# wreuven/h264-scroll-encoder

Hardware: AMD Instinct MI355X
Metric: composed frames/sec (1280x720, 360x360 dyn) at 1/2/4/8 GPU; bit-exact vs CPU (higher is better)
Workload: dtype u8; 1 GPU; BASELINE config 3: 256 concurrent 1280x720 streams + 360x360 synthetic dynamic rect (4x4 int transform + quant + CAVLC), composer_write_scroll_frame semantics; resolution=1280x720, streams_per_gpu=256, parallelism=static stream shard x1, no RCCL

## Files before the change

h264-scroll-encoder_amd/csrc/dyn_device.h:

```cpp
#ifndef SCROLL_DYN_DEVICE_H
#define SCROLL_DYN_DEVICE_H

#include "qparams.h"
#include "scroll_device.h"

namespace scroll {
namespace dyn {

constexpr int QP_DEFAULT = 26, QP_MIN = 22, QP_MAX = 51, LEVEL_MAX = 2063;
__host__ __device__ constexpr int mf_of(int r, int cls)
{
    constexpr int T[6][3] = {{13107, 5243, 8066}, {11916, 4660, 7490}, {10082, 4194, 6554},
                             {9362, 3647, 5825},  {8192, 3355, 5243},  {7282, 2893, 4559}};
    return T[r][cls];
}
__host__ __device__ constexpr QParams qparams(int qp)
{
    return QParams{mf_of(qp % 6, 0), mf_of(qp % 6, 1), mf_of(qp % 6, 2), 15 + qp / 6, (1 << (15 + qp / 6)) / 6};
}
__device__ __host__ inline QParams qparams_rt(int qp)
{
    const int r = qp % 6, b = 15 + qp / 6;
    const int m0 = r == 0 ? 13107 : r == 1 ? 11916 : r == 2 ? 10082 : r == 3 ? 9362 : r == 4 ? 8192 : 7282;
    const int m1 = r == 0 ? 5243 : r == 1 ? 4660 : r == 2 ? 4194 : r == 3 ? 3647 : r == 4 ? 3355 : 2893;
// ... 984 lines not shown
    uint32_t m = (t1 == 0 ? g0 : (t1 == 1 ? g1 : (t1 == 2 ? g2 : g3))) >> 1;
    auto push = [](uint64_t &ac, uint32_t &n, uint32_t v, uint32_t len, CAP &c) {
        if (n + len > 64u) {
            if (n > 32u) c.put((uint32_t)(ac >> 32), (int)(n - 32u));
            c.put((uint32_t)ac, n > 32u ? 32 : (int)n);
            ac = 0;
            n = 0;
        }
        ac = (ac << len) | v;
        n += len;
    };
    int cls = ((tc > 10 && t1 < 3) ? 1 : 0) + (t1 < 3 ? 7 : 0);
    auto level_code = [&](int v, int cl) -> uint32_t {
        if (v >= -LVT_V && v <= LVT_V) return lvt[cl * LVT_W + v + LVT_V + 1];
        const int sl = cl >= 7 ? cl - 7 : cl, adj = cl >= 7 ? 2 : 0;
        const int a = v < 0 ? -v : v;
        const int code = 2 * a - 2 + (v < 0 ? 1 : 0) - adj;
        const int lim = sl ? (15 << sl) : 30;
        const uint32_t mk = (1u << sl) - 1u;
        uint32_t fv = ((uint32_t)code & mk) | (mk + 1u);
        uint32_t fl = (uint32_t)((code >> sl) + 1 + sl);
        const bool e15 = code >= lim, e14 = sl == 0 && code >= 14;
        fv = e15 ? (uint32_t)(4096 + code - lim) : (e14 ? (uint32_t)(code + 2) : fv);
        fl = e15 ? 28u : (e14 ? 19u : fl);
        const int s1 = sl == 0 ? 1 : sl;
        return fv | fl << 13 | (uint32_t)(s1 + ((a > (3 << (s1 - 1)) && s1 < 6) ? 1 : 0)) << 18;
    };
#ifndef SCROLL_CAVLC_NOPF
    const uint32_t m0 = m, an0 = an;
    const uint64_t acc0 = acc;
    const int cls0 = cls;
    const CAP cap0 = cap;
    bool big = false;
    int pn = top_bit(m);
    int vn = (int)lb[pn ^ (int)bx];
    for (int k = t1; k < tc; ++k) {
        const int v = vn;
        m &= ~(1u << pn);
        pn = top_bit(m);
        vn = (int)lb[pn ^ (int)bx];
        const int vc = v < -LVT_V ? -LVT_V : (v > LVT_V ? LVT_V : v);
        big |= vc != v;
        const uint32_t e = lvt[cls * LVT_W + vc + LVT_V + 1];
        push(acc, an, e & 0x1fffu, (e >> 13) & 31u, cap);
        cls = (int)(e >> 18);
    }
    if (big) {
        m = m0;
        an = an0;
        acc = acc0;
        cls = cls0;
        cap = cap0;
        for (int k = t1; k < tc; ++k) {
            const int p = top_bit(m);
            m &= ~(1u << p);
            const uint32_t e = level_code((int)lb[p ^ (int)bx], cls);
            push(acc, an, e & 0x1fffu, (e >> 13) & 31u, cap);
            cls = (int)(e >> 18);
        }
    }
#else
    for (int k = t1; k < tc; ++k) {
        const int p = top_bit(m);
        m &= ~(1u << p);
        const uint32_t e = level_code((int)lb[p ^ (int)bx], cls);
        push(acc, an, e & 0x1fffu, (e >> 13) & 31u, cap);
        cls = (int)(e >> 18);
    }
#endif
    const uint32_t tzl = 31u - (uint32_t)__builtin_ctz(tzrb);
    push(acc, an, (tzrb >> 1) >> (31u - tzl), tzl, cap);
    if (cap.n == 0) {
        cap.lo = acc;
        cap.n = an;
        return tc;
    }
    if (an > 32u) cap.put((uint32_t)(acc >> 32), (int)(an - 32u));
    cap.put((uint32_t)acc, an > 32u ? 32 : (int)an);
    ok = cap.n <= 128;
    return tc;
}

template <class CAP, class PT>
__device__ __host__ inline int cavlc_dc4(CAP &cap, const PT &P, const int c[4])
{
    const uint32_t nz = (c[0] != 0 ? 1u : 0u) | (c[1] != 0 ? 2u : 0u) | (c[2] != 0 ? 4u : 0u) |
                        (c[3] != 0 ? 8u : 0u);
    const int tc = __builtin_popcount(nz);
    int t1 = 0;
    bool trail = true;
#pragma unroll
    for (int i = 3; i >= 0; --i) {
        const bool one = c[i] == 1 || c[i] == -1;
        if (c[i] != 0) {
            trail = trail && one && t1 < 3;
            t1 += trail ? 1 : 0;
        }
    }
    {
        const uint32_t e = P.ct[3][4 * tc + t1];
        cap.put(e & 255u, (int)(e >> 8));
    }
    if (tc == 0) return 0;
    int k = 0, sl = 0, zl = 0, pprev = -1;
    uint64_t runs = 0;
    int rn = 0;
    const int hi = top_bit(nz);
    const int tz = hi + 1 - tc;
    zl = tz;
#pragma unroll
    for (int i = 3; i >= 0; --i) {
        const int v = c[i];
        if (v != 0) {
            const int a = v < 0 ? -v : v;
            if (k < t1) {
                cap.put(v < 0 ? 1u : 0u, 1);
            } else {
                int code = 2 * a - 2 + (v < 0 ? 1 : 0);
                if (k == t1 && t1 < 3) code -= 2;
                uint32_t fv;
                int fl;
                level_field_bf(code, sl, fv, fl);
                cap.put(fv, fl);
                if (sl == 0) sl = 1;
                if (a > (3 << (sl - 1)) && sl < 6) sl++;
            }
            if (k > 0 && zl > 0) {
                const int run = pprev - i - 1;
                const uint32_t e = P.rb[(zl < 7 ? zl : 7) - 1][run];
                runs = (runs << (e >> 8)) | (e & 255u);
                rn += (int)(e >> 8);
                zl -= run;
            }
            pprev = i;
            k++;
        }
    }
    if (tc < 4) {
        const uint32_t e = P.tzdc[tc - 1][tz];
        cap.put(e & 255u, (int)(e >> 8));
    }
    cap.put((uint32_t)runs, rn);
    return tc;
}

__device__ __host__ inline bool ep_insert(uint32_t b, int k) { return b <= 3 && k >= 2 && !(k & 1); }

__device__ __host__ inline int blk_raster(int blk)
{
    const int q8 = blk >> 2, q4 = blk & 3;
    return 4 * ((q8 >> 1) * 2 + (q4 >> 1)) + (q8 & 1) * 2 + (q4 & 1);
}

struct Rect {
    int x0, y0, w, h;
};

__device__ __host__ inline uint32_t magic32(uint32_t d) { return d <= 1 ? 0u : 0xffffffffu / d + 1u; }
__device__ __host__ inline uint32_t div_m(uint32_t x, uint32_t m) { return m ? __umulhi(x, m) : x; }
__device__ __host__ inline uint32_t magic16(uint32_t d) { return (65536u + d - 1u) / d; }
__device__ __host__ inline uint32_t div16(uint32_t x, uint32_t m16) { return __umul24(x, m16) >> 16; }

__device__ __host__ inline int dyn_rank(const Rect &r, int mbw, int m)
{
    const int y = m / mbw, x = m - y * mbw;
    if (y < r.y0) return 0;
    if (y >= r.y0 + r.h) return r.w * r.h;
    return (y - r.y0) * r.w + clampi(x - r.x0, 0, r.w);
}

__device__ __host__ inline int dyn_rank_m(const Rect &r, int mbw, uint32_t m_mbw, int m)
{
    const int y = (int)div_m((uint32_t)m, m_mbw), x = m - y * mbw;
    if (y < r.y0) return 0;
    if (y >= r.y0 + r.h) return r.w * r.h;
    return (y - r.y0) * r.w + clampi(x - r.x0, 0, r.w);
}

__device__ __host__ inline int dyn_mb_m(const Rect &r, int mbw, uint32_t m_rw, int q)
{
    const int ry = (int)div_m((uint32_t)q, m_rw);
    return (r.y0 + ry) * mbw + r.x0 + (q - ry * r.w);
}

__device__ __host__ inline int dyn_mb(const Rect &r, int mbw, int q)
{
    const int ry = q / r.w;
    return (r.y0 + ry) * mbw + r.x0 + (q - ry * r.w);
}

}
}
#endif
```

h264-scroll-encoder_amd/csrc/dyn_kernels.hip:

```cpp
#include <hip/hip_runtime.h>

#include <stdint.h>
#include <mutex>

#include "dyn_device.h"
#include "dyn_engine.h"
#include "nal_ctx.h"
#include "row_mfma.h"
#include "stage_util.h"

using namespace scroll;
using namespace scroll::dyn;
using namespace scroll::stage;

namespace {

__constant__ Tabs g_tabs = SCROLL_DYN_TABS;
constexpr Tabs k_tabs = SCROLL_DYN_TABS;
__constant__ PTabs g_ptabs = make_ptabs(k_tabs);
__device__ uint32_t g_tzrb[TZRB_N];
__constant__ LvTab g_lvt = make_lvt();

struct QpPair {
    QParams l, c;
// ... 376 lines not shown
        const uint16_t mm = ok ? (uint16_t)(cap.n | (uint32_t)tc << 8 | (uint32_t)t1 << 13)
                               : (uint16_t)((uint32_t)tc << 8 | (uint32_t)t1 << 13 | M_OVF);
        M[tk] = mm;
        uint4 ov = v4;
        if (wide && !ok) {
            const uint4 *l2 = reinterpret_cast<const uint4 *>(lw[u]);
            ov = l2[0];
            BW[tk] = l2[1];
        }
        if ((mm & 255u) || (mm & M_OVF))
            put_body(BL, BH, tk,
                     ok ? make_uint4((uint32_t)cap.lo, (uint32_t)(cap.lo >> 32), (uint32_t)cap.hi,
                                     (uint32_t)(cap.hi >> 32))
                        : ov,
                     (mm & 255u) > 64u || (mm & M_OVF));
    }
}

#ifndef SCROLL_CODE_GEN_Y
#define SCROLL_CODE_GEN_Y 64
#endif
constexpr int CODE_GEN_Y = SCROLL_CODE_GEN_Y;
__global__ __launch_bounds__(CODE_T) void k_dyn_code_general(const DevStream *__restrict__ st,
                                                             const DynFrame *__restrict__ dfr, int ld_fr,
                                                             const PlanPending *__restrict__ pend,
                                                             const NalDesc *__restrict__ nal, int ld_nal,
                                                             DynGeom g, const uint32_t *__restrict__ rows,
                                                             const uint8_t *__restrict__ src,
                                                             const uint8_t *__restrict__ refs,
                                                             uint16_t *__restrict__ meta,
                                                             uint2 *__restrict__ blo, uint2 *__restrict__ bhi,
                                                             uint4 *__restrict__ bwd, const uint32_t *__restrict__ ctr)
{
    const uint32_t n = min(__builtin_amdgcn_readfirstlane(ctr[1]), g.gen_cap);
    for (uint32_t j = blockIdx.y; j < n; j += gridDim.y) {
        const uint32_t q = __builtin_amdgcn_readfirstlane(ctr[DYN_CTR_LIST + j]);
        const int s = (int)(q / (uint32_t)ld_fr), f = (int)(q - (uint32_t)s * (uint32_t)ld_fr);
        code_frame(st, dfr, ld_fr, pend, nal, ld_nal, g, rows, src, refs, meta, blo, bhi, bwd, s, f, blockIdx.x);
        __syncthreads();
    }
}

struct LdsOrWin {
    uint32_t *b;
    uint32_t lo, n;
    __device__ inline void operator()(uint32_t i, uint32_t v) const
    {
        const uint32_t k = i - lo;
        if (k < n) atomicOr(&b[k], v);
    }
};
typedef OrSink<LdsOrWin> WSink;


__device__ inline int tc_of(uint32_t m) { return (int)((m >> 8) & 31u); }

struct HeadCtx {
    Regions rg;
    int a_end, mbw, nrefs;
    __device__ inline int sel(int row, int col) const
    {
        const bool curA = row < a_end, abvA = (row - 1) < a_end;
        return 3 * (row == 0 ? 0 : (curA ? 1 : (abvA ? 2 : 3))) + (col == 0 ? 0 : (col == mbw - 1 ? 2 : 1));
    }
    template <class S>
    __device__ inline void put_class(S &sk, int cls) const
    {
        const int ty = cls / 3, pos = cls - 3 * ty;
        const int x = pos == 0 ? 0 : (pos == 1 ? min(1, mbw - 1) : mbw - 1);
        const bool cur = ty == 0 ? 0 < a_end : ty == 1;
        const bool abv = ty == 1 || ty == 2;
        const int ref = cur ? rg.ra : rg.rb, mv4 = 4 * (cur ? rg.mva : rg.mvb);
        const int aref = abv ? rg.ra : rg.rb, amv4 = 4 * (abv ? rg.mva : rg.mvb);
        int px, py;
        predict(x, ty == 0 ? 0 : 1, mbw, ref, mv4, aref, amv4, px, py);
        put_mb_head(sk, ref, 0 - px, mv4 - py, nrefs);
    }
    template <class S>
    __device__ inline void put_slow(S &sk, int row, int col) const
    {
        const bool curA = row < a_end, abvA = (row - 1) < a_end;
        const int ref = curA ? rg.ra : rg.rb, mv4 = 4 * (curA ? rg.mva : rg.mvb);
        const int aref = abvA ? rg.ra : rg.rb, amv4 = 4 * (abvA ? rg.mva : rg.mvb);
        int px, py;
        predict(col, row, mbw, ref, mv4, aref, amv4, px, py);
        put_mb_head(sk, ref, 0 - px, mv4 - py, nrefs);
    }
};

__device__ inline HeadCtx head_ctx(const NalCtx &c)
{
    HeadCtx H;
    H.rg = regions(c);
    H.a_end = (c.h - c.off) / 16;
    H.mbw = c.w / 16;
    H.nrefs = 2 + c.nwp;
    return H;
}

__device__ inline uint32_t row_static_bits(const HeadCtx &H, const uint32_t *hlen, int row, const Rect &R)
{
    const int mbw = H.mbw;
    const bool in = row >= R.y0 && row < R.y0 + R.h;
    auto isdyn = [&](int col) { return in && col >= R.x0 && col < R.x0 + R.w; };
    const int base = H.sel(row, 0) - 0;
    uint32_t bits = isdyn(0) ? 0u : hlen[base] + 1u;
    if (mbw >= 2) {
        if (!isdyn(mbw - 1)) bits += hlen[base + 2] + 1u;
        int nmid = mbw - 2;
        if (in) nmid -= max(0, min(R.x0 + R.w, mbw - 1) - max(R.x0, 1));
        bits += (uint32_t)nmid * (hlen[base + 1] + 1u);
    }
    return bits;
}

__device__ inline void lb_store(unsigned long long *p, uint64_t v)
{
    __hip_atomic_store(p, v, __ATOMIC_RELAXED, __HIP_MEMORY_SCOPE_AGENT);
}

__host__ __device__ inline uint64_t rs_group_words(const DynGeom &g, int nA, int gi)
{
    if (gi < nA) return (uint64_t)gi * g.rs_static_words;
    if (gi < nA + g.h) return (uint64_t)nA * g.rs_static_words + (uint64_t)(gi - nA) * g.rs_row_words;
    return (uint64_t)(gi - g.h) * g.rs_static_words + (uint64_t)g.h * g.rs_row_words;
}

__host__ __device__ inline uint64_t rs_runs_words(const DynGeom &g, int nA, int gi)
{
    const bool row = gi >= nA && gi < nA + g.h;
    return rs_group_words(g, nA, gi) + (row ? g.rs_row_words - EPC_ROW : g.rs_static_words - EPC_STATIC);
}

constexpr uint32_t LO_LEN = 0x7ffu;

__device__ inline void piece_token(const uint16_t (*ct)[68], uint32_t mv, int nC, uint32_t &tv, uint32_t &tl)
{
    const int tc = tc_of(mv), t1 = (int)((mv >> 13) & 3u);
    if (nC >= 8) {
        tv = tc ? (uint32_t)(((tc - 1) << 2) | t1) : 3u;
        tl = 6;
    } else {
        const uint32_t e = ct[nC < 2 ? 0 : (nC < 4 ? 1 : 2)][4 * tc + t1];
        tv = e & 255u;
        tl = e >> 8;
    }
}

__device__ inline void wave_sync()
{
    __builtin_amdgcn_fence(__ATOMIC_RELEASE, "wavefront");
    __builtin_amdgcn_wave_barrier();
    __builtin_amdgcn_fence(__ATOMIC_ACQUIRE, "wavefront");
}

template <class S>
__device__ inline void ovf_code(S &sk, const PTabs &PT, const Tabs &TB, uint4 bd, const uint4 *bw, int pc, int nC)
{
    if (nC == -1) {
        const int dq[4] = {(int)(int16_t)(bd.x & 0xffffu), (int)(int16_t)(bd.x >> 16),
                           (int)(int16_t)(bd.y & 0xffffu), (int)(int16_t)(bd.y >> 16)};
        cavlc_dc4(sk, PT, dq);
    } else if (bw) {
        const uint4 hi = *bw;
        const uint32_t w8[8] = {bd.x, bd.y, bd.z, bd.w, hi.x, hi.y, hi.z, hi.w};
        int16_t l16[16];
#pragma unroll
        for (int i = 0; i < 8; ++i) {
            l16[2 * i] = (int16_t)(w8[i] & 0xffffu);
            l16[2 * i + 1] = (int16_t)(w8[i] >> 16);
        }
        cavlc_block(sk, TB, l16, pc < 16 ? 16 : 15, nC);
    } else {
        const int8_t *lvp = reinterpret_cast<const int8_t *>(&bd);
        cavlc_block(sk, TB, lvp, pc < 16 ? 16 : 15, nC);
    }
}

__device__ __attribute__((noinline)) uint32_t ovf_bits(const PTabs &PT, const Tabs &TB, uint4 bd, const uint4 *bw,
                                                       int pc, int nC)
{
    CountSink cn{0};
    ovf_code(cn, PT, TB, bd, bw, pc, nC);
    return cn.n;
}

__device__ __attribute__((noinline)) void ovf_put(uint32_t *buf, uint32_t lo, uint32_t n, uint32_t pos,
                                                  const PTabs &PT, const Tabs &TB, uint4 bd, const uint4 *bw, int pc,
                                                  int nC)
{
    WSink sk{LdsOrWin{buf, lo, n}, 0, 0, 0};
    sk.start(pos);
    ovf_code(sk, PT, TB, bd, bw, pc, nC);
    sk.finish();
}

__device__ inline uint4 body_msb(uint64_t hi, uint64_t lo, uint32_t n)
{
    const uint32_t k = 128u - n;
    uint64_t H, Lw;
    if (k >= 64u) {
        H = k >= 128u ? 0ull : lo << (k - 64u);
        Lw = 0ull;
    } else {
        H = k ? (hi << k) | (lo >> (64u - k)) : hi;
        Lw = lo << k;
    }
    return make_uint4((uint32_t)(H >> 32), (uint32_t)H, (uint32_t)(Lw >> 32), (uint32_t)Lw);
}

__global__ __launch_bounds__(256) void k_dyn_rows(const DevStream *__restrict__ st,
                                                  const NalDesc *__restrict__ nal, int ld_nal,
                                                  const PlanPending *__restrict__ pend,
                                                  DynFrame *__restrict__ dfr, int ld_fr, DynGeom g,
                                                  uint32_t *__restrict__ rows, uint32_t *__restrict__ ctr,
                                                  uint4 *__restrict__ heads)
{
    __shared__ int32_t wo[8], wl[8], wv[8];
    __shared__ int32_t gen;
    const int s = blockIdx.y, f = blockIdx.x, t = threadIdx.x;
    DynFrame *DF = dfr + (size_t)s * ld_fr + f;
    const int j = DF->nal;
    if (j < 0) return;
    if (t < 8) {
        wo[t] = pend[s].wo[t];
        wl[t] = pend[s].wl[t];
        wv[t] = pend[s].wv[t];
    }
    if (t == 0) gen = 0;
    __syncthreads();
    const DevStream *S = st + s;
    const NalDesc d = nal[(size_t)s * ld_nal + j];
    const NalCtx c = nal_ctx(S, d, wo, wl, wv);
    if (t < 12) {
        const HeadCtx H = head_ctx(c);
        CapSink hc{0, 0, 0};
        H.put_class(hc, t);
        uint4 *hv = heads + ((size_t)s * ld_fr + f) * DYN_HEAD_VECS;
        hv[t] = body_msb(hc.hi, hc.lo, min(hc.n, 128u));
        reinterpret_cast<uint32_t *>(hv + 12)[t] = hc.n | (hc.over() ? 0x80000000u : 0u);
    }
    const Regions rg = regions(c);
    const int w = c.w, h = c.h, a_end = (h - c.off) / 16;
    const uint32_t ysz = (uint32_t)w * (uint32_t)h, pic = ysz + ysz / 2;
    const WpTab T{wo, wv, h};
    uint32_t *rw = rows + ((size_t)s * ld_fr + f) * (size_t)(32 * g.h);
    bool my_gen = false;
    for (int i = t; i < 32 * g.h; i += 256) {
        uint32_t e;
        if (i < 16 * g.h) {
            const int Y = 16 * g.y0 + i, row = Y >> 4;
            const bool cA = row < a_end;
            int yo;
            const int b = luma_row(T, cA ? rg.ra : rg.rb, Y + (cA ? rg.mva : rg.mvb), yo);
            e = (uint32_t)b * pic + (uint32_t)yo * (uint32_t)w;
        } else {
            const int i2 = i - 16 * g.h, bot = i2 >= 8 * g.h;
            const int Y = 8 * g.y0 + (bot ? i2 - 8 * g.h : i2), row = Y >> 3;
            const bool cA = row < a_end;
            const int q = 4 * (cA ? rg.mva : rg.mvb), o = q >> 3, fr = q & 7;
            int yo;
            const int b = chroma_row(T, cA ? rg.ra : rg.rb, Y + o + bot, yo);
            if (b < 0) {
                e = ROW_GEN;
                if (!bot || fr) my_gen = true;
            } else {
                e = ((uint32_t)b * pic + ysz + (uint32_t)yo * (uint32_t)(w / 2)) | (uint32_t)fr << 28;
            }
        }
        rw[i] = e;
    }
    if (my_gen || S->dyn_qp < QP_MIN) gen = 1;
    __syncthreads();
    if (t == 0) {
        uint32_t e = 0u;
        if (gen) {
            const uint32_t k = atomicAdd(&ctr[1], 1u);
            if (k < g.gen_cap) {
                DF->rbsp_bytes = k;
                ctr[DYN_CTR_LIST + k] = (uint32_t)((size_t)s * ld_fr + f);
                e = DF_GENERAL;
            } else {
                e = DF_OVER;
            }
        }
        DF->err = e;
        DF->ep = 0u;
    }
}

constexpr int GW = 64;
#ifndef SCROLL_GBUF_WORDS
#define SCROLL_GBUF_WORDS 256
#endif
constexpr int GBUF_WORDS = SCROLL_GBUF_WORDS;

#ifndef SCROLL_STATIC_WORDS
#define SCROLL_STATIC_WORDS 1
#endif

struct StaticFixed {
    uint32_t ncand;
    uint32_t buf[GBUF_WORDS];
    uint64_t hhi[12], hlo[12];
    uint4 pat[12];
    uint32_t hlen[12];
// ... 781 lines not shown
            if (ok && (e & 3) == 0) {
                const int k = e >> 3, p = (e >> 2) & 1;
                const int q0 = quant_dc(d0 + d1 + d2 + d3, qc), q1 = quant_dc(d0 - d1 + d2 - d3, qc);
                const int q2 = quant_dc(d0 + d1 - d2 - d3, qc), q3 = quant_dc(d0 - d1 - d2 + d3, qc);
                lv[k * NPC + 16 + p] = make_uint4(((uint32_t)q0 & 0xffffu) | (uint32_t)q1 << 16,
                                                  ((uint32_t)q2 & 0xffffu) | (uint32_t)q3 << 16, 0u, 0u);
                mt[k * NPC + 16 + p] = (uint16_t)((uint32_t)((q0 != 0) + (q1 != 0) + (q2 != 0) + (q3 != 0)) << 8);
            }
#endif
        };
        BlkPix A = nx, B;
        int q = 0;
        for (; q + 1 < qL; q += 2) {
            issue_l(q + 1, B);
            code_l(q, A);
            issue_any(q + 2, A);
            code_l(q + 1, B);
        }
        if (q < qL) {
            issue_any(q + 1, B);
            code_l(q, A);
            A = B;
            ++q;
        }
        for (; q + 1 < qC; q += 2) {
            issue_c(q + 1, B);
            code_c(q, A);
            issue_c(q + 2, A);
            code_c(q + 1, B);
        }
        if (q < qC) code_c(q, A);
        (void)np;
#else
        const int qL = nl > wv0 ? (nl - wv0 + T - 1) / T : 0;
        const int qC = ntv > wv0 ? (ntv - wv0 + T - 1) / T : 0;
        const int gq = lane >> 4, ln = lane & 15;
        auto issue_l = [&](int q, MPix &px) { mfetch_pass(mo, false, (uint32_t)((q - mo.pb) * T), fs, rb, px); };
        auto issue_c = [&](int q, MPix &px) {
            if (!mo_chroma) {
                mfetch_chroma(mo, q * T + wv0 - L0, r, g, csz, L.rt + 16, L.rt + 24, lane);
                mo.pb = q;
                mo_chroma = true;
            }
            mfetch_pass(mo, true, (uint32_t)((q - mo.pb) * T), fs, rb, px);
        };
        auto issue_any = [&](int q, MPix &px) {
            if (q < qL) issue_l(q, px);
            else issue_c(q, px);
        };
        auto put_rec = [&](int slot, const uint32_t pk[4]) {
            const uint4 p4 = make_uint4(pk[0], pk[1], pk[2], pk[3]);
            const uint32_t nz = nz_mask16(p4);
            const int n = __builtin_popcount(nz);
            lv[slot] = p4;
            mt[slot] = (uint16_t)nz;
#ifndef SCROLL_ROW_RANK_ALL
            if (n)
#endif
                lo[slot] = (uint16_t)atomicAdd(&L.kc[0][SORT_KEYS - 1 - min(n, SORT_KEYS - 1)], 1u);
        };
        const uint64_t aL = g_kmat.a[0][lane];
        const MQuant QL = mquant_of(gq, true, ql);
        auto code_l = [&](int q, const MPix &px) {
            uint32_t wd[4];
            {
                const mfma_v4i d0 = mtile(aL, px.s.x, px.p.x), d1 = mtile(aL, px.s.y, px.p.y);
                mquant2(d0, d1, QL, wd[0], wd[1]);
            }
            {
                const mfma_v4i d2 = mtile(aL, px.s.z, px.p.z), d3 = mtile(aL, px.s.w, px.p.w);
                mquant2(d2, d3, QL, wd[2], wd[3]);
            }
            mtranspose(wd);
            const int k = ((q * T + wv0) >> 4) + (ln >> 2);
            if (k < w) put_rec((int)__umul24((uint32_t)k, (uint32_t)NPC) + 4 * (ln & 3) + gq, wd);
        };
        auto code_c = [&](int q, const MPix &px, uint64_t aC, const MQuant &QC) {
            uint32_t pr[4];
            const uint32_t up[4] = {px.p.x, px.p.y, px.p.z, px.p.w}, dn[4] = {px.q.x, px.q.y, px.q.z, px.q.w};
            if (frc == 4u) {
#pragma unroll
                for (int j = 0; j < 4; ++j) pr[j] = __builtin_amdgcn_lerp(up[j], dn[j], 0x01010101u);
            } else if (frc == 0u) {
#pragma unroll
                for (int j = 0; j < 4; ++j) pr[j] = up[j];
            } else {
#pragma unroll
                for (int j = 0; j < 4; ++j) pr[j] = bilin4(up[j], dn[j], frc);
            }
            const mfma_v4i d0 = mtile(aC, px.s.x, pr[0]), d1 = mtile(aC, px.s.y, pr[1]);
            const mfma_v4i d2 = mtile(aC, px.s.z, pr[2]), d3 = mtile(aC, px.s.w, pr[3]);
            const int kb = ((q * T + wv0 - L0) >> 3) + 2 * (ln & 3), pl = ln >> 3, by = (ln >> 2) & 1;
            if (gq == 3) {
                const int dcv[4] = {d0[3], d1[3], d2[3], d3[3]};
#pragma unroll
                for (int j = 0; j < 4; ++j) {
                    const int k = kb + (j >> 1);
                    if (k < w)
                        reinterpret_cast<int16_t *>(lv + (int)__umul24((uint32_t)k, (uint32_t)NPC) + 16 + pl)[2 * by + (j & 1)] =
                            (int16_t)dcv[j];
                }
            }
            uint32_t wd[4];
            mquant2(d0, d1, QC, wd[0], wd[1]);
            mquant2(d2, d3, QC, wd[2], wd[3]);
            mtranspose(wd);
            const int k = kb + (gq >> 1);
            if (k < w) put_rec((int)__umul24((uint32_t)k, (uint32_t)NPC) + 18 + 4 * pl + 2 * by + (gq & 1), wd);
        };
        MPix A = mx, B;
        int q = 0;
        for (; q + 1 < qL; q += 2) {
            issue_l(q + 1, B);
            code_l(q, A);
            issue_any(q + 2, A);
            code_l(q + 1, B);
        }
        if (q < qL) {
            issue_any(q + 1, B);
            code_l(q, A);
            A = B;
            ++q;
        }
        if (q < qC) {
            const uint64_t aC = g_kmat.a[1][lane];
            const MQuant QC = mquant_of(gq, false, qc);
            for (; q + 1 < qC; q += 2) {
                issue_c(q + 1, B);
                code_c(q, A, aC, QC);
                issue_c(q + 2, A);
                code_c(q + 1, B, aC, QC);
            }
            if (q < qC) code_c(q, A, aC, QC);
        }
        (void)np;
#endif
        __syncthreads();
        if (stp) stp[1] = __builtin_amdgcn_s_memrealtime();
        const bool nopub = (g.debug & SCROLL_DEBUG_DYN_NOPUBLISH) && s == 0 && f == 0 && r == 0;
        if (t < w && r + 1 < R.h && !nopub) {
            const uint16_t *mk = mt + t * NPC;
            uint64_t v = 0;
#pragma unroll
            for (int e = 0; e < 8; ++e) {
                const int pcA = e < 4 ? 12 + e : (e < 6 ? 16 + e : 18 + e);
#ifdef SCROLL_ROW_OLDREC
                v |= (uint64_t)(tc_of(mk[pcA]) & 31) << (5 * e);
#else
                v |= (uint64_t)__builtin_popcount(mk[pcA]) << (5 * e);
#endif
            }
            lb_store(tcx + (nb * R.h + r) * (size_t)w + t, (uint64_t)(epoch & 0xffffffu) << 40 | v);
        }
        if (t >= T - 2 * w) {
            const int i = t - (T - 2 * w), k = i >> 1, p = i & 1, sl = k * NPC + 16 + p;
            const uint4 q = lv[sl];
#ifdef SCROLL_ROW_OLDREC
            const int dq[4] = {(int)(int16_t)(q.x & 0xffffu), (int)(int16_t)(q.x >> 16),
                               (int)(int16_t)(q.y & 0xffffu), (int)(int16_t)(q.y >> 16)};
#else
            const int d0 = (int)(int16_t)(q.x & 0xffffu), d1 = (int)(int16_t)(q.x >> 16);
            const int d2 = (int)(int16_t)(q.y & 0xffffu), d3 = (int)(int16_t)(q.y >> 16);
            const int dq[4] = {quant_dc(d0 + d1 + d2 + d3, qc), quant_dc(d0 - d1 + d2 - d3, qc),
                               quant_dc(d0 + d1 - d2 - d3, qc), quant_dc(d0 - d1 - d2 + d3, qc)};
#endif
            CapSink cap{0, 0, 0};
            const int tc = cavlc_dc4(cap, L.ptabs, dq);
            if (cap.n <= 128) {
                mt[sl] = (uint16_t)(cap.n | (uint32_t)tc << 8);
                lv[sl] = body_msb(cap.hi, cap.lo, cap.n);
            } else {
                mt[sl] = (uint16_t)((uint32_t)tc << 8 | M_OVF);
#ifndef SCROLL_ROW_OLDREC
                lv[sl] = make_uint4(((uint32_t)dq[0] & 0xffffu) | (uint32_t)dq[1] << 16,
                                    ((uint32_t)dq[2] & 0xffffu) | (uint32_t)dq[3] << 16, 0u, 0u);
#endif
            }
        }
        if (t < SORT_KEYS) {
            const uint32_t tot = L.kc[0][t];
            uint32_t kb = tot;
#pragma unroll
            for (int dd = 1; dd < 32; dd <<= 1) {
                const uint32_t o = __shfl_up(kb, dd, 64);
                if (lane >= dd) kb += o;
            }
            L.kc[1][t] = kb - tot;
        }
        __syncthreads();
        for (int task = t; task < ntask; task += T) {
            const int slot = row_slot(task, w);
#ifdef SCROLL_ROW_OLDREC
            const int tcs = tc_of(mt[slot]);
#else
            const int tcs = __builtin_popcount(mt[slot]);
#endif
            if (tcs) {
                order[L.kc[1][SORT_KEYS - 1 - min(tcs, SORT_KEYS - 1)] + lo[slot]] =
                    (uint16_t)(slot | (task < 16 * w ? 0 : 0x8000));
#if SCROLL_LV_SWZ
                const uint32_t key = lv_key(slot);
                if (key) lv[slot] = lv_swz(lv[slot], key);
#endif
            }
        }
        __syncthreads();
    ROW_CUT(1);
        const int zbase = (int)L.kc[1][SORT_KEYS - 1];
        for (int pa = 0; pa < np; ++pa) {
            const int pos = pa * T + t;
            if (pos >= zbase) continue;
            const uint32_t oe = order[pos];
            const int slot = (int)(oe & 0x7fffu);
            const bool luma = !(oe & 0x8000u);
            CapSink cap{0, 0, 0};
            int t1 = 0;
            bool ok = true;
#ifdef SCROLL_ROW_OLDREC
            const uint32_t nz = nz_mask16(lv[slot]);
#else
            const uint32_t nz = mt[slot];
#endif
            const uint32_t tzrb = g_tzrb[luma ? nz : 65536u + nz];
            const uint32_t key = SCROLL_LV_SWZ ? lv_key(slot) : 0u;
            const int tc = cavlc_body_t(cap, reinterpret_cast<const int8_t *>(lv + slot), nz, tzrb, t1, ok, L.lvt,
                                        key << 2);
            mt[slot] = ok ? (uint16_t)(cap.n | (uint32_t)tc << 8 | (uint32_t)t1 << 13)
                          : (uint16_t)((uint32_t)tc << 8 | (uint32_t)t1 << 13 | M_OVF);
            if (ok) lv[slot] = body_msb(cap.hi, cap.lo, cap.n);
            else if (key) lv[slot] = lv_swz(lv[slot], key);
        }
    } else {
        const int q0 = r * w;
        const size_t gs = df.rbsp_bytes;
        const uint16_t *M = meta + gs * (size_t)(NPC * ndt);
        const uint2 *BL = blo + gs * (size_t)(NPC * ndt), *BH = bhi + gs * (size_t)(NPC * ndt);
        for (int i = t; i < npc; i += T) {
            const int k = div_npc(i), pc = i - k * NPC;
            const int rec = rec_of(q0 + k, pc, ndt);
            const uint16_t mv = M[rec];
            mt[i] = mv;
            uint4 bv = make_uint4(0u, 0u, 0u, 0u);
            if ((mv & 255u) || (mv & M_OVF)) {
                const uint4 bd = get_body(BL, BH, rec, (mv & 255u) > 64u || (mv & M_OVF));
                bv = (mv & M_OVF) ? bd
                                  : body_msb((uint64_t)bd.z | (uint64_t)bd.w << 32,
                                             (uint64_t)bd.x | (uint64_t)bd.y << 32, mv & 255u);
            }
            lv[i] = bv;
        }
        for (int i = t; i < 8 * w; i += T) {
            const int k = i >> 3, e = i & 7;
            const int pcA = e < 4 ? 12 + e : (e < 6 ? 16 + e : 18 + e);
            ta[i] = r > 0 ? (uint8_t)tc_of(M[rec_of(q0 + k - w, pcA, ndt)]) : (uint8_t)0;
        }
    }
    if (!general && wave == nwv - 1) {
        uint64_t prev = r > 0 ? __builtin_amdgcn_s_memrealtime() : 0ull, waited = 0;
        bool late = false;
        for (int k = lane; k < w; k += 64) {
            uint64_t v = 0;
            if (r > 0) {
                const unsigned long long *p = tcx + (nb * R.h + r - 1) * (size_t)w + k;
                for (;;) {
                    v = __hip_atomic_load(p, __ATOMIC_RELAXED, __HIP_MEMORY_SCOPE_AGENT);
                    if ((uint32_t)(v >> 40) == (epoch & 0xffffffu)) break;
                    const uint64_t now = __builtin_amdgcn_s_memrealtime(), gap = now - prev;
                    prev = now;
                    if (gap < HANDOFF_GAP) waited += gap;
                    if (waited > HANDOFF_TICKS) {
                        v = 0;
                        late = true;
                        break;
                    }
                    __builtin_amdgcn_s_sleep(1);
                }
            }
#pragma unroll
            for (int e = 0; e < 8; ++e) ta[8 * k + e] = (uint8_t)((v >> (5 * e)) & 31u);
        }
        if (__builtin_amdgcn_ballot_w64(late) != 0 && lane == 0) atomicOr(&dfr[nb].err, DF_HANDOFF);
    }
    const NalCtx c = nal_ctx(S, d, L.wo, L.wl, L.wv);
    const HeadCtx H = head_ctx(c);
    const bool wide = GEN && __builtin_amdgcn_readfirstlane(S->dyn_qp) < QP_MIN;
    auto ovf_wide = [&](int k, int pc) -> const uint4 * {
        if (!wide) return nullptr;
        return bwd + (size_t)df.rbsp_bytes * (size_t)(NPC * ndt) + rec_of(r * w + k, pc, ndt);
    };
    __syncthreads();
    if (stp) stp[2] = __builtin_amdgcn_s_memrealtime();
    ROW_CUT(2);

    const Tabs &TB = g_tabs;
    const PTabs &PT = *reinterpret_cast<const PTabs *>(&g_ptabs);
    const uint16_t(*ctab)[68] = L.ptabs.ct;
    const int nAe = R.x0 > 0 ? 0 : -1, nBe = row > 0 ? 0 : -1;
    auto token = [&](int i, int k, int pc, uint32_t D) {
        const uint32_t mv = mt[i];
        const int ia = max(i + (int)(D & 63u) - 32, 0), ib = max(i + (int)((D >> 7) & 63u) - 32, 0);
        const int tA = tc_of(mt[ia]), tB = tc_of(mt[ib]), tT = (int)ta[8 * k + (int)((D >> 14) & 7u)];
        const int nA = ((D & 64u) && k == 0) ? nAe : tA;
        const int nB = (D & 8192u) ? (r > 0 ? tT : nBe) : tB;
        const int mean = (nA + nB + 1) >> 1, one = max(max(nA, nB), 0);
        const int nC0 = (nA | nB) >= 0 ? mean : one;
        const int nC = (D >> 17) ? -1 : nC0;
        const int tc = tc_of(mv), t1 = (int)((mv >> 13) & 3u);
        const uint32_t ce = ctab[nC < 0 ? 3 : (nC < 2 ? 0 : (nC < 4 ? 1 : 2))][4 * tc + t1];
        const uint32_t tl = nC < 0 ? 0u : (nC >= 8 ? 6u : ce >> 8);
        uint32_t len = tl + (mv & 255u);
        if (mv & M_OVF) len = ovf_bits(PT, TB, lv[i], ovf_wide(k, pc), pc, nC);
        uint32_t nc1 = (uint32_t)(nC + 1);
        if (!(mv & M_OVF) && nC >= 0 && len <= 128u) {
            const uint32_t tv = nC >= 8 ? (tc ? (uint32_t)(((tc - 1) << 2) | t1) : 3u) : (ce & 255u);
            const uint32_t tw = tv & low_mask((int)tl);
            const uint4 b = lv[i];
            lv[i] = make_uint4(__builtin_amdgcn_alignbit(tw, b.x, tl), __builtin_amdgcn_alignbit(b.x, b.y, tl),
                               __builtin_amdgcn_alignbit(b.y, b.z, tl), __builtin_amdgcn_alignbit(b.z, b.w, tl));
            mt[i] = (uint16_t)((mv & ~255u) | len);
            nc1 = 0u;
        }
        lo[i] = (uint16_t)(len | nc1 << 11);
    };
    for (int i = t; i < npc; i += T) {
        const int k = div_npc(i), pc = i - k * NPC;
        token(i, k, pc, L.pcd[pc]);
    }
    __syncthreads();
    if (stp) stp[3] = __builtin_amdgcn_s_memrealtime();
    ROW_CUT(3);
    const bool head_over = L.head_over;
    auto head_bits = [&](int rr, int col) -> uint32_t {
        if (!head_over) return L.hlen[H.sel(rr, col)];
        CountSink cn{0};
        H.put_slow(cn, rr, col);
        return cn.n;
    };

    for (int k = t; k < w; k += T) {
        const uint16_t *mk = mt + k * NPC;
        int cbp_l = 0;
#pragma unroll
        for (int pc = 0; pc < 16; ++pc)
            if (tc_of(mk[pc])) cbp_l |= 1 << (2 * (pc >> 3) + ((pc & 3) >> 1));
        bool ac = false;
#pragma unroll
        for (int pc = 18; pc < NPC; ++pc) ac |= tc_of(mk[pc]) != 0;
        const bool dc = (tc_of(mk[16]) | tc_of(mk[17])) != 0;
        const int cbp_c = ac ? 2 : (dc ? 1 : 0);
        const int cbp = cbp_l | cbp_c << 4;
        const int code = TB.cbp_code[cbp];
        CountSink hs{head_bits(row, R.x0 + k)};
        put_ue(hs, (uint32_t)code);
        if (cbp) put_se(hs, 0);
        uint32_t off = hs.n;
        const uint16_t *lk = lo + k * NPC;
        uint16_t *ok = off16 + k * NPC;
#pragma unroll
        for (int blk = 0; blk < 16; ++blk) {
            const int rr = blk_raster(blk);
            const bool pres = (cbp_l >> (blk >> 2)) & 1;
            ok[rr] = pres ? (uint16_t)off : (uint16_t)0xffffu;
            off += pres ? (lk[rr] & LO_LEN) : 0u;
        }
#pragma unroll
        for (int k2 = 16; k2 < NPC; ++k2) {
            const bool pres = k2 < 18 ? cbp_c >= 1 : cbp_c == 2;
            ok[k2] = pres ? (uint16_t)off : (uint16_t)0xffffu;
            off += pres ? (lk[k2] & LO_LEN) : 0u;
        }
        mbits[k] = off;
        cbpa[k] = (uint8_t)cbp;
        codea[k] = (uint8_t)code;
    }
    const int x1 = R.x0 + w;
    const uint32_t h0 = head_bits(row, 0) + 1u;
    const uint32_t h1 = mbw >= 3 ? head_bits(row, 1) + 1u : 0u;
    const uint32_t h2 = mbw >= 2 ? head_bits(row, mbw - 1) + 1u : 0u;
    auto colpos = [&](int col) -> uint32_t {
        if (col <= R.x0) return col == 0 ? 0u : h0 + (uint32_t)(col - 1) * h1;
        if (col < x1) return moff[col - R.x0];
        return moff[w] + (uint32_t)(col - x1) * h1 + (col == mbw && x1 <= mbw - 1 ? h2 - h1 : 0u);
    };
    __syncthreads();
    const int gi = nA + r;
    if (wave == 0) {
        uint32_t carry = R.x0 == 0 ? 0u : h0 + (uint32_t)(R.x0 - 1) * h1;
        for (int k0 = 0; k0 < w; k0 += 64) {
            const int k = k0 + lane;
            const uint32_t len = k < w ? mbits[k] : 0u;
            const uint32_t incl = wave_incl_sum(len, lane);
            if (k < w) moff[k] = carry + incl - len;
            carry += __shfl(incl, 63, 64);
        }
        if (lane == 0) moff[w] = carry;
    }
    __syncthreads();
    if (stp) stp[4] = __builtin_amdgcn_s_memrealtime();
    ROW_CUT(4);
    const uint32_t bits = colpos(mbw);
    if (t == 0) gbits[nb * (size_t)ng + gi] = bits;

    const bool wwin = row_wide_win(w);
    uint32_t *const wb = wwin ? reinterpret_cast<uint32_t *>(reinterpret_cast<uint8_t *>(rdyn) + row_wide_off(w)) : L.buf;
    const uint32_t GBW = wwin ? (uint32_t)ROW_GB_WIDE : (uint32_t)ROW_GB;
    uint32_t *out = rowstage + nb * g.rs_frame_words + rs_group_words(g, nA, gi);
    uint32_t epc = g.rs_row_words - EPC_ROW;
    bool lost = false;
    if (((bits + 31u) >> 5) > epc) {
        if (t == 0) L.spill = atomicAdd(&ctr[0], 1u);
        __syncthreads();
        const uint32_t k = L.spill;
        uint32_t *fr = rowstage + nb * g.rs_frame_words;
        uint32_t *sp = spill + (size_t)k * g.rs_spill_words;
        if (k >= g.rs_spill_cap || (uint64_t)(sp - fr) + g.rs_spill_words > 0x3fffffffull) {
            if (t == 0) atomicOr(&dfr[nb].err, DF_OVER);
            lost = true;
        } else {
            if (t == 0) out[epc] = 0x80000000u | (uint32_t)(sp - fr);
            out = sp;
            epc = g.rs_spill_words - EPC_ROW;
        }
    }
    const uint32_t nw = lost ? 0u : min((bits + 31u) >> 5, epc);
    const int npass = (int)((nw + GBW - 1) / GBW);
    for (int pi = 0; pi < npass; ++pi) {
        const uint32_t p0 = (uint32_t)pi * GBW;
        const uint32_t n = min((uint32_t)GBW, nw - p0);
        for (uint32_t i = (uint32_t)t; i < n; i += (uint32_t)T) wb[i] = 0u;
        __syncthreads();
        const LdsOrWin win{wb, p0, n};
        const bool one = npass == 1;
        for (int col = t; col < mbw; col += T) {
            const uint32_t pos = colpos(col);
            if (!one && (pos >= 32u * (p0 + n) || colpos(col + 1) <= 32u * p0)) continue;
            const int k = col - R.x0;
            const bool in = k >= 0 && k < w;
            if (one && !head_over) {
                const int cls = H.sel(row, col);
                const uint32_t hl = L.hlen[cls];
                uint32_t tv = 1u, tn = 1u;
                if (in) {
                    const uint32_t x = (uint32_t)codea[k] + 1u, lz = 31u - (uint32_t)__builtin_clz(x);
                    tv = x;
                    tn = 2u * lz + 1u;
                    if (cbpa[k]) {
                        tv = tv << 1 | 1u;
                        ++tn;
                    }
                }
                if (hl + tn <= 128u) {
                    const uint64_t ha = L.hhi[cls], hb = L.hlo[cls];
                    const uint32_t t32 = tv << (32u - tn), q = hl >> 5, r = hl & 31u;
                    uint32_t wv[4] = {(uint32_t)(ha >> 32), (uint32_t)ha, (uint32_t)(hb >> 32), (uint32_t)hb};
#pragma unroll
                    for (uint32_t j = 0; j < 4; ++j)
                        wv[j] |= (j == q ? t32 >> r : 0u) | (j == q + 1u && r ? t32 << (32u - r) : 0u);
                    put_piece1(wb, pos, 0u, 0u, make_uint4(wv[0], wv[1], wv[2], wv[3]), hl + tn);
                    continue;
                }
            }
            WSink sk{win, 0, 0, 0};
            sk.start(pos);
            if (!head_over) {
                const int cls = H.sel(row, col);
                sk.put_cap(cap_of_msb(L.hhi[cls], L.hlo[cls], L.hlen[cls]));
            } else {
                H.put_slow(sk, row, col);
            }
            if (!in) {
                sk.put(1, 1);
            } else {
                put_ue(sk, (uint32_t)codea[k]);
                if (cbpa[k]) put_se(sk, 0);
            }
            sk.finish();
        }
        for (int i = t; i < npc; i += T) {
            const uint32_t o = off16[i];
            if (o == 0xffffu) continue;
            const int k = div_npc(i), pc = i - k * NPC;
            const uint32_t e = lo[i], mv = mt[i];
            const uint32_t pos = moff[k] + o;
            if (!one && (pos >= 32u * (p0 + n) || pos + (e & LO_LEN) <= 32u * p0)) continue;
            const int nC = (int)(e >> 11) - 1;
            const uint4 bd = lv[i];
            if (!(mv & M_OVF)) {
                if (nC == -1) {
                    if (one) put_piece1(wb, pos, 0u, 0u, bd, mv & 255u);
                    else put_piece(wb, p0, n, pos, 0u, 0u, bd, mv & 255u);
                } else {
                    uint32_t tv = 0, tl = 0;
                    piece_token(ctab, mv, nC, tv, tl);
                    if (one) put_piece1(wb, pos, tv, tl, bd, mv & 255u);
                    else put_piece(wb, p0, n, pos, tv, tl, bd, mv & 255u);
                }
            } else {
                ovf_put(wb, p0, n, pos, PT, TB, bd, ovf_wide(k, pc), pc, nC);
            }
        }
        __syncthreads();
        flush_window(wb, n, p0, p0 + n >= nw, out, &L.ncand, out + epc, EPC_ROW - 1, t, T);
        __syncthreads();
    }
    if (t == 0 && !lost) out[epc] = L.ncand;
    if (stp) {
        stp[5] = __builtin_amdgcn_s_memrealtime();
        stp[6] = bits;
        stp[7] = (uint64_t)(uint32_t)__builtin_amdgcn_s_getreg((31 << 11) | 4);
    }
}

#ifndef SCROLL_EPS_KW
#define SCROLL_EPS_KW 4
#endif
constexpr int EPS_KW = SCROLL_EPS_KW;
static_assert(EPS_KW % 4 == 0, "the EP scan reads 16-byte LDS vectors");
__host__ __device__ inline size_t gtab_bytes(int ng, bool epfix)
{
    return (size_t)4 * (epfix ? 5 * (size_t)ng + 2 : 3 * (size_t)ng + 1);
}
struct GTab {
    uint32_t *goff, *gb, *gw, *cw, *cbase;
};
__device__ inline GTab gtab_of(uint32_t *p, int ng)
{
    GTab T;
    T.goff = p;
    T.gb = p + ng + 1;
    T.gw = T.gb + ng;
    T.cw = T.gw + ng;
    T.cbase = T.cw + ng;
    return T;
}

__device__ inline uint32_t rs_word_span(uint32_t P, int &gg, int ng, uint32_t T, const uint32_t *goff,
                                       const uint32_t *gb, const uint32_t *gw, const uint32_t *fr)
{
    uint32_t acc = 0, filled = 0;
    while (filled < 32u && gg < ng && P + filled < T) {
        const uint32_t lp = P + filled - goff[gg];
        if (lp >= gb[gg]) {
            ++gg;
            continue;
        }
        const uint32_t take = min(32u - filled, gb[gg] - lp);
        const uint32_t *src = fr + gw[gg];
        const uint32_t i = lp >> 5, sh = lp & 31u;
        uint32_t x = src[i];
        if (sh) {
// ... 1408 lines not shown
```

Before: 2.811 million frames/s.

## Parallelize per-MB CBP/offset computation across lanes with DPP scans

Replaces the one-thread-per-macroblock loop that computes CBP, header bits and per-block bit offsets with an 8-lanes-per-macroblock scheme. It uses ballot for the CBP bits, a shuffle table lookup for the CBP code and a DPP segmented prefix sum for the offsets. Shuffle-based scans are swapped for DPP row-shift scans, and for narrow rows the moff scan runs redundantly in every wave with a wave sync instead of a block barrier. The chroma-DC CAVLC pass moves after the token pass, and a __syncthreads before the sort is replaced by a wave-level sync. The aim is to cut barriers and serial per-thread work, at the cost of subtle lane-mapping and synchronization correctness risks.

```diff
diff --git a/h264-scroll-encoder_amd/csrc/dyn_device.h b/h264-scroll-encoder_amd/csrc/dyn_device.h
--- a/h264-scroll-encoder_amd/csrc/dyn_device.h
+++ b/h264-scroll-encoder_amd/csrc/dyn_device.h
@@ -1160,6 +1160,8 @@
     return 4 * ((q8 >> 1) * 2 + (q4 >> 1)) + (q8 & 1) * 2 + (q4 & 1);
 }
 
+__device__ __host__ inline uint32_t ue_bits(uint32_t v) { return 2u * (31u - (uint32_t)__builtin_clz(v + 1u)) + 1u; }
+
 struct Rect {
     int x0, y0, w, h;
 };
diff --git a/h264-scroll-encoder_amd/csrc/dyn_kernels.hip b/h264-scroll-encoder_amd/csrc/dyn_kernels.hip
--- a/h264-scroll-encoder_amd/csrc/dyn_kernels.hip
+++ b/h264-scroll-encoder_amd/csrc/dyn_kernels.hip
@@ -552,6 +552,29 @@
     __builtin_amdgcn_fence(__ATOMIC_RELEASE, "wavefront");
     __builtin_amdgcn_wave_barrier();
     __builtin_amdgcn_fence(__ATOMIC_ACQUIRE, "wavefront");
+}
+
+template <int CTRL, int ROWS>
+__device__ inline uint32_t dpp_or0(uint32_t v)
+{
+    return (uint32_t)__builtin_amdgcn_update_dpp(0, (int)v, CTRL, ROWS, 0xf, false);
+}
+
+__device__ inline uint32_t seg32_incl_sum(uint32_t v)
+{
+    v += dpp_or0<0x111, 0xf>(v);
+    v += dpp_or0<0x112, 0xf>(v);
+    v += dpp_or0<0x114, 0xf>(v);
+    v += dpp_or0<0x118, 0xf>(v);
+    v += dpp_or0<0x142, 0xa>(v);
+    return v;
+}
+
+__device__ inline uint32_t wave_incl_sum_dpp(uint32_t v)
+{
+    v = seg32_incl_sum(v);
+    v += dpp_or0<0x143, 0xc>(v);
+    return v;
 }
 
 template <class S>
@@ -1639,42 +1662,16 @@
             }
             lb_store(tcx + (nb * R.h + r) * (size_t)w + t, (uint64_t)(epoch & 0xffffffu) << 40 | v);
         }
-        if (t >= T - 2 * w) {
-            const int i = t - (T - 2 * w), k = i >> 1, p = i & 1, sl = k * NPC + 16 + p;
-            const uint4 q = lv[sl];
-#ifdef SCROLL_ROW_OLDREC
-            const int dq[4] = {(int)(int16_t)(q.x & 0xffffu), (int)(int16_t)(q.x >> 16),
-                               (int)(int16_t)(q.y & 0xffffu), (int)(int16_t)(q.y >> 16)};
-#else
-            const int d0 = (int)(int16_t)(q.x & 0xffffu), d1 = (int)(int16_t)(q.x >> 16);
-            const int d2 = (int)(int16_t)(q.y & 0xffffu), d3 = (int)(int16_t)(q.y >> 16);
-            const int dq[4] = {quant_dc(d0 + d1 + d2 + d3, qc), quant_dc(d0 - d1 + d2 - d3, qc),
-                               quant_dc(d0 + d1 - d2 - d3, qc), quant_dc(d0 - d1 - d2 + d3, qc)};
-#endif
-            CapSink cap{0, 0, 0};
-            const int tc = cavlc_dc4(cap, L.ptabs, dq);
-            if (cap.n <= 128) {
-                mt[sl] = (uint16_t)(cap.n | (uint32_t)tc << 8);
-                lv[sl] = body_msb(cap.hi, cap.lo, cap.n);
-            } else {
-                mt[sl] = (uint16_t)((uint32_t)tc << 8 | M_OVF);
-#ifndef SCROLL_ROW_OLDREC
-                lv[sl] = make_uint4(((uint32_t)dq[0] & 0xffffu) | (uint32_t)dq[1] << 16,
-                                    ((uint32_t)dq[2] & 0xffffu) | (uint32_t)dq[3] << 16, 0u, 0u);
-#endif
-            }
-        }
-        if (t < SORT_KEYS) {
-            const uint32_t tot = L.kc[0][t];
+        {
+            const uint32_t tot = lane < SORT_KEYS ? L.kc[0][lane] : 0u;
             uint32_t kb = tot;
-#pragma unroll
-            for (int dd = 1; dd < 32; dd <<= 1) {
-                const uint32_t o = __shfl_up(kb, dd, 64);
-                if (lane >= dd) kb += o;
-            }
-            L.kc[1][t] = kb - tot;
-        }
-        __syncthreads();
+            kb += dpp_or0<0x111, 0xf>(kb);
+            kb += dpp_or0<0x112, 0xf>(kb);
+            kb += dpp_or0<0x114, 0xf>(kb);
+            kb += dpp_or0<0x118, 0xf>(kb);
+            if (lane < SORT_KEYS) L.kc[1][lane] = kb - tot;
+            wave_sync();
+        }
         for (int task = t; task < ntask; task += T) {
             const int slot = row_slot(task, w);
 #ifdef SCROLL_ROW_OLDREC
@@ -1716,6 +1713,32 @@
                           : (uint16_t)((uint32_t)tc << 8 | (uint32_t)t1 << 13 | M_OVF);
             if (ok) lv[slot] = body_msb(cap.hi, cap.lo, cap.n);
             else if (key) lv[slot] = lv_swz(lv[slot], key);
+        }
+        const int dcT = nwv > 1 ? T - 64 : T;
+        for (int i = dcT - 1 - t; i >= 0 && i < 2 * w; i += dcT) {
+            const int k = i >> 1, p = i & 1, sl = k * NPC + 16 + p;
+            const uint4 q = lv[sl];
+#ifdef SCROLL_ROW_OLDREC
+            const int dq[4] = {(int)(int16_t)(q.x & 0xffffu), (int)(int16_t)(q.x >> 16),
+                               (int)(int16_t)(q.y & 0xffffu), (int)(int16_t)(q.y >> 16)};
+#else
+            const int d0 = (int)(int16_t)(q.x & 0xffffu), d1 = (int)(int16_t)(q.x >> 16);
+            const int d2 = (int)(int16_t)(q.y & 0xffffu), d3 = (int)(int16_t)(q.y >> 16);
+            const int dq[4] = {quant_dc(d0 + d1 + d2 + d3, qc), quant_dc(d0 - d1 + d2 - d3, qc),
+                               quant_dc(d0 + d1 - d2 - d3, qc), quant_dc(d0 - d1 - d2 + d3, qc)};
+#endif
+            CapSink cap{0, 0, 0};
+            const int tc = cavlc_dc4(cap, L.ptabs, dq);
+            if (cap.n <= 128) {
+                mt[sl] = (uint16_t)(cap.n | (uint32_t)tc << 8);
+                lv[sl] = body_msb(cap.hi, cap.lo, cap.n);
+            } else {
+                mt[sl] = (uint16_t)((uint32_t)tc << 8 | M_OVF);
+#ifndef SCROLL_ROW_OLDREC
+                lv[sl] = make_uint4(((uint32_t)dq[0] & 0xffffu) | (uint32_t)dq[1] << 16,
+                                    ((uint32_t)dq[2] & 0xffffu) | (uint32_t)dq[3] << 16, 0u, 0u);
+#endif
+            }
         }
     } else {
         const int q0 = r * w;
@@ -1809,6 +1832,7 @@
         }
         lo[i] = (uint16_t)(len | nc1 << 11);
     };
+    const uint32_t cbtab = TB.cbp_code[min(lane, 47)];
     for (int i = t; i < npc; i += T) {
         const int k = div_npc(i), pc = i - k * NPC;
         token(i, k, pc, L.pcd[pc]);
@@ -1824,41 +1848,56 @@
         return cn.n;
     };
 
-    for (int k = t; k < w; k += T) {
-        const uint16_t *mk = mt + k * NPC;
-        int cbp_l = 0;
-#pragma unroll
-        for (int pc = 0; pc < 16; ++pc)
-            if (tc_of(mk[pc])) cbp_l |= 1 << (2 * (pc >> 3) + ((pc & 3) >> 1));
-        bool ac = false;
-#pragma unroll
-        for (int pc = 18; pc < NPC; ++pc) ac |= tc_of(mk[pc]) != 0;
-        const bool dc = (tc_of(mk[16]) | tc_of(mk[17])) != 0;
-        const int cbp_c = ac ? 2 : (dc ? 1 : 0);
-        const int cbp = cbp_l | cbp_c << 4;
-        const int code = TB.cbp_code[cbp];
-        CountSink hs{head_bits(row, R.x0 + k)};
-        put_ue(hs, (uint32_t)code);
-        if (cbp) put_se(hs, 0);
-        uint32_t off = hs.n;
-        const uint16_t *lk = lo + k * NPC;
-        uint16_t *ok = off16 + k * NPC;
-#pragma unroll
-        for (int blk = 0; blk < 16; ++blk) {
-            const int rr = blk_raster(blk);
-            const bool pres = (cbp_l >> (blk >> 2)) & 1;
-            ok[rr] = pres ? (uint16_t)off : (uint16_t)0xffffu;
-            off += pres ? (lk[rr] & LO_LEN) : 0u;
-        }
-#pragma unroll
-        for (int k2 = 16; k2 < NPC; ++k2) {
-            const bool pres = k2 < 18 ? cbp_c >= 1 : cbp_c == 2;
-            ok[k2] = pres ? (uint16_t)off : (uint16_t)0xffffu;
-            off += pres ? (lk[k2] & LO_LEN) : 0u;
-        }
-        mbits[k] = off;
-        cbpa[k] = (uint8_t)cbp;
-        codea[k] = (uint8_t)code;
+    {
+        const int j = t & 7, G = T >> 3;
+        const bool lum = j < 4, four = j != 4;
+        const int pb = lum ? 8 * (j >> 1) + 2 * (j & 1) : (j == 4 ? 16 : (j == 5 ? 18 : 22));
+        const int d2 = lum ? 4 : 2, d3 = d2 + 1;
+        for (int k0 = wv0 >> 3; k0 < w; k0 += G) {
+            const int k = k0 + (lane >> 3);
+            const bool live = k < w && j < 7;
+            const int i0 = (int)__umul24((uint32_t)k, (uint32_t)NPC) + pb;
+            uint32_t mm = 0u, l0 = 0u, l1 = 0u, l2 = 0u, l3 = 0u;
+            if (live) {
+                mm = (uint32_t)mt[i0] | mt[i0 + 1];
+                l0 = lo[i0] & LO_LEN;
+                l1 = lo[i0 + 1] & LO_LEN;
+                if (four) {
+                    mm |= (uint32_t)mt[i0 + d2] | mt[i0 + d3];
+                    l2 = lo[i0 + d2] & LO_LEN;
+                    l3 = lo[i0 + d3] & LO_LEN;
+                }
+            }
+            const uint64_t nzw = __builtin_amdgcn_ballot_w64((mm & 0x1f00u) != 0u);
+            const uint32_t m = (uint32_t)(nzw >> (lane & 56)) & 0x7fu;
+            const uint32_t cbp_l = m & 15u, cbp_c = (m & 0x60u) ? 2u : (m >> 4);
+            const uint32_t cbp = cbp_l | cbp_c << 4;
+            const uint32_t code = (uint32_t)__shfl((int)cbtab, (int)cbp, 64);
+            const bool pres = lum ? (m >> j) & 1u : (j == 4 ? cbp_c >= 1u : cbp_c == 2u);
+            const uint32_t tot = pres ? l0 + l1 + l2 + l3 : 0u;
+            uint32_t incl = tot, u;
+            u = dpp_or0<0x111, 0xf>(incl);
+            incl += j >= 1 ? u : 0u;
+            u = dpp_or0<0x112, 0xf>(incl);
+            incl += j >= 2 ? u : 0u;
+            u = dpp_or0<0x114, 0xf>(incl);
+            incl += j >= 4 ? u : 0u;
+            const uint32_t hb = head_bits(row, R.x0 + min(k, w - 1)) + ue_bits(code) + (cbp ? 1u : 0u);
+            const uint32_t o0 = hb + incl - tot, no = pres ? 0u : 0xffffu;
+            if (live) {
+                off16[i0] = (uint16_t)(o0 | no);
+                off16[i0 + 1] = (uint16_t)((o0 + l0) | no);
+                if (four) {
+                    off16[i0 + d2] = (uint16_t)((o0 + l0 + l1) | no);
+                    off16[i0 + d3] = (uint16_t)((o0 + l0 + l1 + l2) | no);
+                }
+            }
+            if (j == 7 && k < w) {
+                mbits[k] = hb + incl;
+                cbpa[k] = (uint8_t)cbp;
+                codea[k] = (uint8_t)code;
+            }
+        }
     }
     const int x1 = R.x0 + w;
     const uint32_t h0 = head_bits(row, 0) + 1u;
@@ -1871,18 +1910,27 @@
     };
     __syncthreads();
     const int gi = nA + r;
-    if (wave == 0) {
-        uint32_t carry = R.x0 == 0 ? 0u : h0 + (uint32_t)(R.x0 - 1) * h1;
-        for (int k0 = 0; k0 < w; k0 += 64) {
-            const int k = k0 + lane;
-            const uint32_t len = k < w ? mbits[k] : 0u;
-            const uint32_t incl = wave_incl_sum(len, lane);
-            if (k < w) moff[k] = carry + incl - len;
-            carry += __shfl(incl, 63, 64);
-        }
-        if (lane == 0) moff[w] = carry;
-    }
-    __syncthreads();
+    const uint32_t mb0 = R.x0 == 0 ? 0u : h0 + (uint32_t)(R.x0 - 1) * h1;
+    if (w <= 64) {
+        const uint32_t len = lane < w ? mbits[lane] : 0u;
+        const uint32_t incl = wave_incl_sum_dpp(len);
+        if (lane < w) moff[lane] = mb0 + incl - len;
+        if (lane == w - 1) moff[w] = mb0 + incl;
+        wave_sync();
+    } else {
+        if (wave == 0) {
+            uint32_t carry = mb0;
+            for (int k0 = 0; k0 < w; k0 += 64) {
+                const int k = k0 + lane;
+                const uint32_t len = k < w ? mbits[k] : 0u;
+                const uint32_t incl = wave_incl_sum_dpp(len);
+                if (k < w) moff[k] = carry + incl - len;
+                carry += __shfl(incl, 63, 64);
+            }
+            if (lane == 0) moff[w] = carry;
+        }
+        __syncthreads();
+    }
     if (stp) stp[4] = __builtin_amdgcn_s_memrealtime();
     ROW_CUT(4);
     const uint32_t bits = colpos(mbw);
```

New measurement: 2.885 million frames/s (median of 6 runs). 1.03x the previous value.
